# lixilinx/psgd_tf

Hardware: AMD Instinct MI355X
Metric: uvd_update_apply_params_per_sec (higher is better)
Workload: dtype f32

## Files before the change

### psgd_tf_amd/csrc/psgd_uvd.hip

```cpp
#include "uvd_kernels.h"
#include "psgd_hip.h"
#include <math.h>

namespace psgd {

const UvdOps* uvd_ops_group0(int r);
const UvdOps* uvd_ops_group1(int r);
const UvdOps* uvd_ops_group2(int r);
const UvdOps* uvd_ops_group3(int r);

const UvdWideOps* uvd_wide_group0(int r);
const UvdWideOps* uvd_wide_group1(int r);
const UvdWideOps* uvd_wide_group2(int r);
const UvdWideOps* uvd_wide_group3(int r);
const UvdWideOps* uvd_wide_ops_for_rank(int r) {
  if (r <= PSGD_UVD_MAX_RANK || r > 2 * PSGD_UVD_MAX_RANK) return nullptr;
  switch ((r - 33) / 8) {
    case 0: return uvd_wide_group0(r);
    case 1: return uvd_wide_group1(r);
    case 2: return uvd_wide_group2(r);
    default: return uvd_wide_group3(r);
  }
}

// ... 42 lines not shown
  double* sums; float* coef; float* maxbuf; void* part; float* pmax; float* nabla;
};

static int ws_open(void* ws, int64_t ws_bytes, int64_t N, int r, Ws* out) {
  if (N <= 0) return PSGD_ERR_BAD_ARG;
  if (r < 1 || r > PSGD_UVD_MAX_RANK) return PSGD_ERR_RANK;
  if (!ws || (reinterpret_cast<uintptr_t>(ws) & 255)) return PSGD_ERR_WORKSPACE;
  const WsLayout L = ws_layout(N, r);
  if (ws_bytes < L.total) return PSGD_ERR_WORKSPACE;
  char* b = static_cast<char*>(ws);
  out->sums = reinterpret_cast<double*>(b + L.sums_off);
  out->coef = reinterpret_cast<float*>(b + L.coef_off);
  out->maxbuf = reinterpret_cast<float*>(b + L.max_off);
  out->part = b + L.part_off;
  out->pmax = reinterpret_cast<float*>(b + L.pmax_off);
  out->nabla = reinterpret_cast<float*>(b + L.nabla_off);
  return PSGD_OK;
}

static inline bool misaligned16(const void* p) { return (reinterpret_cast<uintptr_t>(p) & 15) != 0; }

static int g_tune_staging = 0;
static int g_tune_blocks_per_cu = 0;
static int g_tune_tiles_per_wave = 8;

constexpr int kProfSlots = 8;
constexpr int kProfMaxPairs = 4096;
struct ProfPair { hipEvent_t e0, e1; };
static int g_prof_on = 0;
static ProfPair g_prof_pairs[kProfSlots][kProfMaxPairs];
static int g_prof_created[kProfSlots];
static int g_prof_used[kProfSlots];

struct ProfScope {
  hipEvent_t e1 = nullptr;
  hipStream_t st;
  ProfScope(int slot, hipStream_t s) : st(s) {
    if (!g_prof_on || slot < 0 || slot >= kProfSlots || g_prof_used[slot] >= kProfMaxPairs) return;
    const int i = g_prof_used[slot];
    if (i >= g_prof_created[slot]) {
      if (hipEventCreate(&g_prof_pairs[slot][i].e0) != hipSuccess) return;
      if (hipEventCreate(&g_prof_pairs[slot][i].e1) != hipSuccess) return;
      g_prof_created[slot] = i + 1;
    }
    g_prof_used[slot] = i + 1;
    (void)hipEventRecord(g_prof_pairs[slot][i].e0, st);
    e1 = g_prof_pairs[slot][i].e1;
  }
  ~ProfScope() {
    if (e1) (void)hipEventRecord(e1, st);
  }
};

static int num_cus() {
  static int n = 0;
  if (n == 0) {
    int dev = 0;
    (void)hipGetDevice(&dev);
    int v = 0;
    if (hipDeviceGetAttribute(&v, hipDeviceAttributeMultiprocessorCount, dev) != hipSuccess || v <= 0) v = 256;
    n = v;
  }
  return n;
}

static inline int use_nt(int64_t N, int r) {
  if (g_tune_staging == 1) return 0;
  if (g_tune_staging == 2) return 1;
  return (int64_t)N * r * 8 > (int64_t)192 * 1024 * 1024;
}

int policy_nt(int64_t stream_bytes) {
  if (g_tune_staging == 1) return 0;
  if (g_tune_staging == 2) return 1;
  return stream_bytes > (int64_t)192 * 1024 * 1024;
}
int policy_grid_blocks(int occ) {
  if (occ <= 0) occ = 1;
  if (g_tune_blocks_per_cu > 0 && g_tune_blocks_per_cu < occ) occ = g_tune_blocks_per_cu;
  if (g_tune_blocks_per_cu < 0) occ = -g_tune_blocks_per_cu;
  return occ;
}
int device_cus() { return num_cus(); }

static int g_tune_grid[16] = {0};

static int sweep_grid(const UvdOps* ops, int r, int which, int64_t N, int hard_cap) {
  static int occ_cache[PSGD_UVD_MAX_RANK + 1][16];
  if (which >= 0 && which < 16 && g_tune_grid[which] > 0) {
    const int64_t tiles = (N + ops->tile_rows - 1) / ops->tile_rows;
    int64_t grid = (tiles + kWavesPerBlock - 1) / kWavesPerBlock;
    if (grid > g_tune_grid[which]) grid = g_tune_grid[which];
    if (grid > hard_cap) grid = hard_cap;
    return (int)(grid < 1 ? 1 : grid);
  }
  int occ = occ_cache[r][which];
  if (occ == 0) {
    occ = ops->occupancy(which);
    if (occ <= 0) occ = 1;
    occ_cache[r][which] = occ;
  }
  if (which == kOccUpdS2U || which == kOccUpdS2V || which == kOccUpdS2F) {
    const int want = ((long)ops->tile_rows * r * 4 >= 4096) ? 1 : 2;
    if (want < occ) occ = want;
  } else if (which == kOccFinal) {
    occ = 1;
  }
  if (g_tune_blocks_per_cu > 0 && g_tune_blocks_per_cu < occ) occ = g_tune_blocks_per_cu;
  if (g_tune_blocks_per_cu < 0) occ = -g_tune_blocks_per_cu;
  const int64_t tiles = (N + ops->tile_rows - 1) / ops->tile_rows;
  int64_t grid = (tiles + kWavesPerBlock - 1) / kWavesPerBlock;
  int64_t cap = (int64_t)num_cus() * occ;
  if (g_tune_blocks_per_cu == 0) {
    int64_t want = tiles / (kWavesPerBlock * (g_tune_tiles_per_wave > 0 ? g_tune_tiles_per_wave : 1));
    if (want < num_cus()) want = num_cus();
    if (cap > want) cap = want;
  }
  if (grid > cap) grid = cap;
  if (grid > hard_cap) grid = hard_cap;
  if (grid < 1) grid = 1;
  return (int)grid;
}

template <class T>
__global__ __launch_bounds__(kThreads) void k_reduce_sum(const T* __restrict__ part, int G, int L,
                                                         double* __restrict__ sums, float* __restrict__ coef) {
  __shared__ double red[kWavesPerBlock][64];
  const int lane = threadIdx.x & 63, w = threadIdx.x >> 6;
  const int id = blockIdx.x * 64 + lane;
  double s = 0.0;
  if (id < L) {
    int b = w;
    for (; b + 7 * kWavesPerBlock < G; b += 8 * kWavesPerBlock) {
      T x[8];
#pragma unroll
      for (int u = 0; u < 8; ++u) x[u] = part[(long)(b + u * kWavesPerBlock) * L + id];
#pragma unroll
      for (int u = 0; u < 8; ++u) s += (double)x[u];
    }
    for (; b < G; b += kWavesPerBlock) s += (double)part[(long)b * L + id];
  }
  red[w][lane] = s;
  __syncthreads();
  if (w == 0 && id < L) {
    const double t = ((red[0][lane] + red[1][lane]) + red[2][lane]) + red[3][lane];
    sums[id] = t;
    if (coef) coef[id] = (float)t;
  }
}

__global__ __launch_bounds__(kThreads) void k_reduce_sum_t(const float* __restrict__ part, int G, int L,
                                                           double* __restrict__ sums, float* __restrict__ coef) {
  const int lane = threadIdx.x & 63;
  const int id = blockIdx.x * kWavesPerBlock + (threadIdx.x >> 6);
  if (id >= L) return;
  const float* p = part + (long)id * G;
  float x[kMaxGrid / 64];
#pragma unroll
  for (int u = 0; u < kMaxGrid / 64; ++u) x[u] = p[min(lane + 64 * u, G - 1)];
  double s = 0.0;
#pragma unroll
  for (int u = 0; u < kMaxGrid / 64; ++u) s += (lane + 64 * u < G) ? (double)x[u] : 0.0;
#pragma unroll
  for (int off = 32; off > 0; off >>= 1) s += __shfl_down(s, off, 64);
  if (lane == 0) {
    sums[id] = s;
// ... 655 lines not shown
      for (int off = 32; off > 0; off >>= 1) sum += __shfl_down(sum, off, 64);
      if (lane == 0) { pqs[e] = sum; pq[e] = sum; }
    }
  } else {
    for (int e = tid; e < 4 * r; e += blockDim.x) pqs[e] = pq[e];
    if (tid == 0) mx = maxbuf[0];
  }
  const int nb = (2 * r + 2 + 15) / 16;
  auto Gm = [&](int a, int b) -> double {
    if constexpr (DENSE) return gram[a * (2 * r + 2) + b];
    if (a > b) { const int t = a; a = b; b = t; }
    const int bi = a >> 4, bj = b >> 4, i = a & 15, j = b & 15;
    const int p = bi * nb - (bi * (bi - 1)) / 2 + (bj - bi);
    return gram[p * 256 + (i & 3) * 64 + (((i >> 2) << 4) | j)];
  };
  const bool act = tid < r;
  if (act) {
    for (int j0 = 0; j0 < r; j0 += 8) {
      double t[8];
#pragma unroll
      for (int u = 0; u < 8; ++u) t[u] = Gm(tid, (j0 + u < r) ? j0 + u : 0);
#pragma unroll
      for (int u = 0; u < 8; ++u)
        if (j0 + u < r) A[tid][j0 + u] = t[u];
    }
    if (update_U) {
      const double mu = c64[4 * r], aa = c64[4 * r + 1], ab = c64[4 * r + 2], bb = c64[4 * r + 3];
      const double Ua = c64[tid], Ub = c64[r + tid], c1 = c64[2 * r + tid], c2 = c64[3 * r + tid];
      for (int j = 0; j < r; ++j) {
        const double Uaj = c64[j], Ubj = c64[r + j], c1j = c64[2 * r + j], c2j = c64[3 * r + j];
        A[tid][j] += -mu * (Ua * c1j + c1 * Uaj - Ub * c2j - c2 * Ubj) +
                     mu * mu * (aa * c1 * c1j - ab * (c1 * c2j + c2 * c1j) + bb * c2 * c2j);
      }
    }
  }
  __syncthreads();
  const double mud = (double)(step / (mx + tiny));
  if (act) s1n[tid] = pqs[r + tid] - mud * pqs[3 * r + tid];
  __syncthreads();
  if (act) {
    double s2 = pqs[tid] - mud * pqs[2 * r + tid];
    for (int k = 0; k < r; ++k) s2 += A[tid][k] * s1n[k];
    coef[tid] = (float)s1n[tid];
    coef[r + tid] = (float)s2;
    s_out[tid] = s1n[tid];
    s_out[r + tid] = s2;
  }
}

}

using namespace psgd;

#define PSGD_CHECK_LAUNCH(expr)                 \
  do {                                          \
    const int _e = (expr);                      \
    if (_e != 0) return PSGD_ERR_LAUNCH;        \
  } while (0)

static inline int last_launch() { return (int)hipGetLastError(); }

extern "C" {

int psgd_abi_version(void) { return PSGD_ABI_VERSION; }

const char* psgd_error_string(int code) {
  switch (code) {
    case PSGD_OK: return "ok";
    case PSGD_ERR_BAD_ARG: return "bad argument (null pointer or non-positive size)";
    case PSGD_ERR_RANK: return "rank of modification outside [1, 32]";
    case PSGD_ERR_WORKSPACE: return "workspace missing, too small or not 256-byte aligned";
    case PSGD_ERR_ALIGN: return "matrix pointer not 16-byte aligned";
    case PSGD_ERR_LAUNCH: return "HIP kernel launch failed";
    case PSGD_ERR_SHAPE: return "inconsistent or unsupported matrix shapes";
    default: return "unknown error";
  }
}

int psgd_set_tuning(int key, int value) {
  if (key == 0) { g_tune_staging = value; return PSGD_OK; }
  if (key == 1) { g_tune_blocks_per_cu = value; return PSGD_OK; }
  if (key == 2) { g_tune_coef = value; return PSGD_OK; }
  if (key == 3) { g_tune_tiles_per_wave = value; return PSGD_OK; }
  if (key >= 10 && key < 26) { g_tune_grid[key - 10] = value; return PSGD_OK; }
  return PSGD_ERR_BAD_ARG;
}

int psgd_prof_enable(int on) {
  g_prof_on = on ? 1 : 0;
  for (int s = 0; s < kProfSlots; ++s) g_prof_used[s] = 0;
  return PSGD_OK;
}

int psgd_prof_collect(int slot, double* total_ms, int* count) {
  if (slot < 0 || slot >= kProfSlots || !total_ms || !count) return PSGD_ERR_BAD_ARG;
  double tot = 0.0;
  int n = 0;
  for (int i = 0; i < g_prof_used[slot]; ++i) {
    float ms = 0.0f;
    if (hipEventSynchronize(g_prof_pairs[slot][i].e1) != hipSuccess) continue;
    if (hipEventElapsedTime(&ms, g_prof_pairs[slot][i].e0, g_prof_pairs[slot][i].e1) != hipSuccess) continue;
    tot += ms;
    ++n;
  }
  g_prof_used[slot] = 0;
  *total_ms = tot;
  *count = n;
  return PSGD_OK;
}

int64_t psgd_uvd_workspace_bytes(int64_t N, int r) {
  if (N <= 0) return PSGD_ERR_BAD_ARG;
  if (r < 1 || r > PSGD_UVD_MAX_RANK) return PSGD_ERR_RANK;
  return ws_layout(N, r).total;
}

int psgd_uvd_ws_region(int which, int stage, int64_t N, int r, int64_t* offset_bytes, int64_t* count) {
  if (!offset_bytes || !count || N <= 0) return PSGD_ERR_BAD_ARG;
  if (r < 1 || r > PSGD_UVD_MAX_RANK) return PSGD_ERR_RANK;
  const WsLayout L = ws_layout(N, r);
  const int nc = 2 * r + 2, nb = (nc + 15) / 16, np = nb * (nb + 1) / 2;
  if (which == PSGD_WS_SUMS_F64) {
    if (stage == 1) { *offset_bytes = L.sums_off; *count = r; return PSGD_OK; }
    if (stage == 2) { *offset_bytes = L.sums_off + (int64_t)r * 8; *count = r; return PSGD_OK; }
    if (stage == 11) { *offset_bytes = L.sums_off; *count = (int64_t)np * 256; return PSGD_OK; }
    if (stage == 13) { *offset_bytes = L.sums_off + (int64_t)kPqSumsOff * 8; *count = 4 * r; return PSGD_OK; }
  } else if (which == PSGD_WS_MAX_F32) {
    if (stage == 10) { *offset_bytes = L.max_off; *count = 2; return PSGD_OK; }
    if (stage == 12) { *offset_bytes = L.max_off + 8; *count = 1; return PSGD_OK; }
  } else if (which == PSGD_WS_SEND_F64) {
    if (stage == 1 || stage == 2 || stage == 11) return psgd_uvd_ws_region(PSGD_WS_SUMS_F64, stage, N, r, offset_bytes, count);
    if (stage == 10) { *offset_bytes = L.sums_off + (int64_t)kBalD64Off * 8; *count = 2; return PSGD_OK; }
    if (stage == 12) { *offset_bytes = L.sums_off + (int64_t)(kPqSumsOff + 4 * r) * 8; *count = 1; return PSGD_OK; }
    if (stage == 13) { *offset_bytes = L.sums_off + (int64_t)kPqSumsOff * 8; *count = 4 * r + 1; return PSGD_OK; }
  }
  return PSGD_ERR_BAD_ARG;
}

int psgd_uvd_fold_gathered_f64(int stage, const double* gathered, int world, int64_t N, int r, void* ws,
                               int64_t ws_bytes, void* stream) {
  if (!gathered || world < 1) return PSGD_ERR_BAD_ARG;
  Ws w;
  const int rc = ws_open(ws, ws_bytes, N, r, &w);
  if (rc) return rc;
  int64_t off = 0, count = 0;
  const int rr = psgd_uvd_ws_region(PSGD_WS_SEND_F64, stage, N, r, &off, &count);
  if (rr) return rr;
  double* dst = reinterpret_cast<double*>(static_cast<char*>(ws) + off);
  int nsum = (int)count;
  float* maxdst = nullptr;
  if (stage == 10) { nsum = 0; maxdst = w.maxbuf; }
  else if (stage == 12) { nsum = 0; maxdst = w.maxbuf + 2; }
  else if (stage == 13) { nsum = 4 * r; maxdst = w.maxbuf + 2; }
  hipLaunchKernelGGL(k_fold_gathered, dim3(((int)count + 255) / 256), dim3(256), 0, static_cast<hipStream_t>(stream),
                     gathered, world, (int)count, nsum, dst, maxdst);
  PSGD_CHECK_LAUNCH(last_launch());
  return PSGD_OK;
}

int psgd_uvd_apply_sweep1_f32(const float* V, const float* d, const float* g, int64_t N, int r, void* ws,
                              int64_t ws_bytes, void* stream) {
  if (!V || !d || !g) return PSGD_ERR_BAD_ARG;
  Ws w;
  const int rc = ws_open(ws, ws_bytes, N, r, &w);
  if (rc) return rc;
  if (misaligned16(V)) return PSGD_ERR_ALIGN;
// ... 688 lines not shown
```

### psgd_tf_amd/csrc/uvd_kernels.h

```cpp
#pragma once
#include <hip/hip_runtime.h>
#include <stdint.h>
#include <type_traits>
#include "nanmax.h"

namespace psgd {

constexpr int kWave = 64;
constexpr int kWavesPerBlock = 4;
constexpr int kThreads = kWave * kWavesPerBlock;
constexpr int kMaxGrid = 2048;
constexpr int kGramMaxGrid = 1024;
#ifndef PSGD_TILE_CHUNK
#define PSGD_TILE_CHUNK 1
#endif
constexpr int kTileChunk = PSGD_TILE_CHUNK;

typedef float f32x4 __attribute__((ext_vector_type(4)));

#ifndef PSGD_WAVE_ID_VGPR
__device__ __forceinline__ int wave_in_block() { return __builtin_amdgcn_readfirstlane((int)(threadIdx.x >> 6)); }
#else
__device__ __forceinline__ int wave_in_block() { return (int)(threadIdx.x >> 6); }
#endif
// ... 862 lines not shown
    sweep_rows<R, 2, NV, (UPDATE_U ? 0 : 1), NT>(mats, vecs, UPDATE_U ? U : V, N, lds, body);
  }
  block_max_store(vmax, red, part_max + blockIdx.x);
}

template <int R, bool NT>
__global__ __launch_bounds__(kThreads) void k_uvd_final(const float* U, const float* V, float* d, const float* nabla,
                                                        const float* g, float* out, long N,
                                                        const float* __restrict__ coef, const float* __restrict__ maxbuf,
                                                        float step, float tiny) {
  __shared__ __attribute__((aligned(16))) float lds[kWavesPerBlock][sweep_lds_floats<R, 2, 3>()];
  const float mu = step / (maxbuf[0] + tiny);
  const float* const mats[2] = {U, V};
  const float* const vecs[3] = {d, nabla, g};
  sweep_rows<R, 2, 3, -1, NT>(mats, vecs, nullptr, N, lds[wave_in_block()],
                              [&](long row, bool valid, float (&x)[2][R], float (&s)[3]) {
                                const float dn = s[0] - (mu * s[0]) * s[1];
                                const float g1 = dn * s[2] + dot_row<R>(x[0], coef);
                                const float o = dn * (g1 + dot_row<R>(x[1], coef + R));
                                if (valid) {
                                  stream_store<NT>(d + row, dn);
                                  stream_store<NT>(out + row, o);
                                }
                              });
}

template <int R, bool NT, bool STR = false>
__global__ __launch_bounds__(kThreads) void k_rank2_update(float* M, const float* a, const float* b, long N,
                                                           const float* __restrict__ coef, long ld = R) {
  __shared__ __attribute__((aligned(16))) float lds[kWavesPerBlock][sweep_lds_floats<R, 1, 2>()];
  const float* const mats[1] = {M};
  const float* const vecs[2] = {a, b};
  sweep_rows<R, 1, 2, 0, NT, STR>(mats, vecs, M, N, lds[wave_in_block()],
                                  [&](long, bool, float (&x)[1][R], float (&s)[2]) {
#pragma unroll
                                    for (int c = 0; c < R; ++c) x[0][c] = x[0][c] - (s[0] * coef[c] - s[1] * coef[R + c]);
                                  }, NoTileHook(), RowStrides{{ld, ld}});
}

struct UvdOps {
  int tile_rows;
  int gram_len;
  int (*colreduce)(int nt, int nvec, const float* M, const float* a, const float* b, long N, float* part, int grid, hipStream_t st);
  int (*apply_s2)(int nt, const float* U, const float* d, const float* g, float* g1out, long N, const float* coef, float* part, int grid, hipStream_t st);
  int (*apply_s3)(int nt, const float* V, const float* d, float* out, long N, const float* coef, int grid, hipStream_t st);
  int (*rowdot_axpy)(int nt, const float* M, const float* x, float* out, long N, const float* coef, int grid, hipStream_t st);
  int (*update_gram)(int nt, const float* U, const float* V, const float* d, const float* v, const float* h, long N, double* part, int grid, hipStream_t st);
  int (*update_s2)(int nt, int update_U, float* U, float* V, const float* d, const float* v, const float* h, const float* g, long N, const float* coef, float* nabla, float* part_max, double* part_pq, int grid, hipStream_t st);
  int (*colreduce4)(int nt, const float* M, const float* const* x, long N, double* part, int grid, hipStream_t st);
  int (*rowdot_axpy4)(int nt, const float* M, const float* const* x, float* const* o, int ncols, long N, const float* coef, int grid, hipStream_t st);
  int (*rank2_update)(int nt, float* M, const float* a, const float* b, long N, const float* coef, int grid, hipStream_t st);
  int (*final_sweep)(int nt, const float* U, const float* V, float* d, const float* nabla, const float* g, float* out, long N, const float* coef, const float* maxbuf, float step, float tiny, int grid, hipStream_t st);
  int (*apply4_s1)(int nt, const float* V, const float* d, const float* const* x, long N, double* part, int grid, hipStream_t st);
  int (*apply4_s2)(int nt, const float* U, const float* d, const float* const* x, float* const* o, int ncols, long N, const float* coef, double* part, int grid, hipStream_t st);
  int (*apply4_s3)(int nt, const float* V, const float* d, float* const* o, int ncols, long N, const float* coef, int grid, hipStream_t st);
  int load_vec;
  int (*update_gram_ld)(const float* U, long ldU, const float* V, long ldV, const float* d, const float* v, const float* h, long N, double* part, int grid, hipStream_t st);
  int (*colreduce4_ld)(const float* M, long ld, const float* const* x, long N, double* part, int grid, hipStream_t st);
  int (*rowdot_axpy4_ld)(const float* M, long ld, const float* const* x, float* const* o, int ncols, long N, const float* coef, int grid, hipStream_t st);
  int (*rank2_update_ld)(float* M, long ld, const float* a, const float* b, long N, const float* coef, int grid, hipStream_t st);
  int (*occupancy)(int which);
};

struct UvdWideOps {
  int tile_rows;
  int (*colreduce4)(int nt, const float* M, const float* const* x, long N, double* part, int grid, hipStream_t st);
  int (*rowdot_axpy4)(int nt, const float* M, const float* const* x, float* const* o, int ncols, long N, const float* coef, int grid, hipStream_t st);
  int (*rank2_update)(int nt, float* M, const float* a, const float* b, long N, const float* coef, int grid, hipStream_t st);
  int (*apply4_s1)(int nt, const float* V, const float* d, const float* const* x, long N, double* part, int grid, hipStream_t st);
  int (*apply4_s2)(int nt, const float* U, const float* d, const float* const* x, float* const* o, int ncols, long N, const float* coef, double* part, int grid, hipStream_t st);
  int (*apply4_s3)(int nt, const float* V, const float* d, float* const* o, int ncols, long N, const float* coef, int grid, hipStream_t st);
  int (*update_s2)(int nt, int update_U, float* U, float* V, const float* d, const float* v, const float* h, const float* g, long N, const float* coef, float* nabla, float* part_max, double* part_pq, int grid, hipStream_t st);
  int (*final_sweep)(int nt, const float* U, const float* V, float* d, const float* nabla, const float* g, float* out, long N, const float* coef, const float* maxbuf, float step, float tiny, int grid, hipStream_t st);
};
const UvdWideOps* uvd_wide_ops_for_rank(int r);

enum { kOccColreduce = 0, kOccApplyS2, kOccApplyS3, kOccRowdot, kOccGram, kOccUpdS2U, kOccUpdS2V, kOccUpdS2F, kOccFinal };

const UvdOps* uvd_ops_for_rank(int r);

int policy_nt(int64_t stream_bytes);
int policy_grid_blocks(int occupancy);
int device_cus();

}
```

### psgd_tf_amd/csrc/uvd_wide_gram.hip

```cpp
#include "uvd_kernels.h"

#include "psgd_hip.h"

#include <cstdlib>

namespace psgd {

#ifndef GW_ACC64_LDS
#define GW_ACC64_LDS 0
#endif
#ifndef GW_DBG
#define GW_DBG 0
#endif
constexpr int kGwRows = 32;
constexpr int kGwThreads = 1024;
constexpr int kGwMulWaves = 11;
constexpr int kGwDepth = 4;

__host__ __device__ constexpr int gw_pair_index(int NB, int bi, int bj) { return bi * NB - (bi * (bi - 1)) / 2 + (bj - bi); }

struct GwPlan {
  int owner[15];
  int slot0[15];
  int max_load;
  int base[kGwMulWaves];
  int load[kGwMulWaves];
};
template <int NB>
constexpr GwPlan gw_make_plan() {
  constexpr int NS = (NB + 1) / 2, NSP = NS * (NS + 1) / 2;
  GwPlan p{};
  int load[kGwMulWaves] = {};
  int wt[15] = {};
  bool placed[15] = {};
  for (int si = 0; si < NS; ++si)
    for (int sj = si; sj < NS; ++sj) {
      const int na = (NB - 2 * si) < 2 ? (NB - 2 * si) : 2, nb = (NB - 2 * sj) < 2 ? (NB - 2 * sj) : 2;
      wt[gw_pair_index(NS, si, sj)] = si == sj ? na * (na + 1) / 2 : na * nb;
    }
  for (int round = 0; round < NSP; ++round) {
    int best = -1;
    for (int sp = 0; sp < NSP; ++sp)
      if (!placed[sp] && (best < 0 || wt[sp] > wt[best])) best = sp;
    int w = 0;
    for (int k = 1; k < kGwMulWaves; ++k)
      if (load[k] < load[w]) w = k;
    p.owner[best] = w;
    p.slot0[best] = load[w];
    load[w] += wt[best];
    placed[best] = true;
  }
  for (int k = 0; k < kGwMulWaves; ++k)
    if (load[k] > p.max_load) p.max_load = load[k];
  for (int k = 0, b = 0; k < kGwMulWaves; ++k) { p.base[k] = b; p.load[k] = load[k]; b += load[k]; }
  return p;
}
template <int NB> struct GwPlanOf { static constexpr GwPlan value = gw_make_plan<NB>(); };

template <int N> struct GwInt { static constexpr int value = N; };
template <int I, int N, class F>
__device__ __forceinline__ void gw_static_for(F&& f) {
  if constexpr (I < N) {
    f(GwInt<I>{});
    gw_static_for<I + 1, N>(f);
  }
}

#ifndef GW_UNIT_COLMAJOR
template <int NC> __device__ __forceinline__ int gw_unit(int col, int rg) { return rg * NC + col; }
#else
template <int NC> __device__ __forceinline__ int gw_unit(int col, int rg) { return col * 4 + (rg ^ ((col >> 2) & 2)); }
#endif

template <int NB, bool NT, bool TAIL>
__global__ __launch_bounds__(kGwThreads) void k_gram_wide(const float* __restrict__ U, const float* __restrict__ V,
                                                          const float* __restrict__ d, const float* __restrict__ v,
                                                          const float* __restrict__ h, long N, int r, long ntiles, long tile0,
                                                          double* __restrict__ part) {
  constexpr int NC = NB * 16;
  constexpr int NPW = GwPlanOf<NB>::value.max_load;
  constexpr int NP = NB * (NB + 1) / 2;
  typedef unsigned int u32x4g __attribute__((ext_vector_type(4)));
  __shared__ __attribute__((aligned(16))) u32x4g PL[2][3][NC * 4 + 16];
#if GW_ACC64_LDS
  __shared__ double A64[NP][4][64];
#endif
  const int tid = threadIdx.x, lane = tid & 63, wave = tid >> 6;
  const long G = gridDim.x;
  const long tfirst = TAIL ? tile0 : (long)blockIdx.x;
  if (TAIL) ntiles = tile0 + 1;

  const long nmine = (ntiles - tfirst + G - 1) / G;
  const long tlast = tfirst + (nmine - 1) * G;
  auto clampt = [&](long t) { return t < tlast ? t : tlast; };
  auto tile_loop = [&](auto&& prologue, auto&& step) {
    __syncthreads();
    prologue();
    __syncthreads();
    for (long i = 0; i < nmine; i += kGwDepth)
      gw_static_for<0, kGwDepth>([&](auto ic) {
        step(ic, tfirst + (i + decltype(ic)::value) * G);
        __syncthreads();
      });
  };
  if (wave < 4) {
    const int col = tid % r, g0 = tid / r;
    const bool on = g0 < 4;
    const unsigned e0 = on ? (unsigned)(g0 * 8 * r + col) : 0u;
    const unsigned eb0 = e0 * 4u;
    const int un0 = gw_unit<NC>(col, on ? g0 : 0), un1 = gw_unit<NC>(r + col, on ? g0 : 0);
    for (int i = tid; i < 2 * 3 * (NC * 4 + 16); i += 256) (&PL[0][0][0])[i] = u32x4g{0u, 0u, 0u, 0u};
    float px[kGwDepth][16];
    auto fetch = [&](long t, auto ic) {
      constexpr int ib = decltype(ic)::value;
      if constexpr (!TAIL) {
        const long toff0 = t * kGwRows * r;
        const long toff = ((long)__builtin_amdgcn_readfirstlane((int)(toff0 >> 32)) << 32) |
                          (unsigned)__builtin_amdgcn_readfirstlane((int)toff0);
        const unsigned tbytes = (unsigned)(kGwRows * r * 4);
        const auto ru = __builtin_amdgcn_make_buffer_rsrc(const_cast<float*>(U + toff), 0, tbytes, 0x00020000);
        const auto rv = __builtin_amdgcn_make_buffer_rsrc(const_cast<float*>(V + toff), 0, tbytes, 0x00020000);
        constexpr int aux = NT ? 2 : 0;
#pragma unroll
        for (int j = 0; j < 8; ++j) {
          px[ib][j] = __builtin_bit_cast(float, __builtin_amdgcn_raw_buffer_load_b32(ru, eb0, j * r * 4, aux));
          px[ib][8 + j] = __builtin_bit_cast(float, __builtin_amdgcn_raw_buffer_load_b32(rv, eb0, j * r * 4, aux));
        }
      } else {
        const long row0 = t * kGwRows + (on ? g0 : 0) * 8;
#pragma unroll
        for (int j = 0; j < 8; ++j) {
          const long row = row0 + j, rc = (row < N ? row : N - 1) * r + col;
          const float xu = stream_load<NT>(U + rc), xv = stream_load<NT>(V + rc);
          px[ib][j] = (on && row < N) ? xu : 0.0f;
          px[ib][8 + j] = (on && row < N) ? xv : 0.0f;
        }
      }
    };
    auto split_to = [&](int buf, auto ic) {
      constexpr int ib = decltype(ic)::value;
      if (GW_DBG & 4) {
#pragma unroll
        for (int j = 0; j < 16; ++j) asm volatile("" ::"v"(px[ib][j]));
        return;
      }
      if (!on) return;
      bf16x8 fh, fm, fl;
      float x[8];
#pragma unroll
      for (int hh = 0; hh < 2; ++hh) {
#pragma unroll
        for (int j = 0; j < 8; ++j) x[j] = px[ib][hh * 8 + j];
        split3_bf16(x, fh, fm, fl);
        const int un = hh ? un1 : un0;
        PL[buf][0][un] = __builtin_bit_cast(u32x4g, fh);
        PL[buf][1][un] = __builtin_bit_cast(u32x4g, fm);
        PL[buf][2][un] = __builtin_bit_cast(u32x4g, fl);
      }
    };
    const long t0 = tfirst;
    tile_loop(
        [&]() {
          gw_static_for<0, kGwDepth>([&](auto ic) { fetch(clampt(t0 + decltype(ic)::value * G), ic); });
          split_to(0, GwInt<0>{});
          fetch(clampt(t0 + kGwDepth * G), GwInt<0>{});
        },
        [&](auto ic, long t) {
          constexpr int q = decltype(ic)::value, slot = (q + 1) % kGwDepth;
          split_to((q + 1) & 1, GwInt<slot>{});
          fetch(clampt(t + (1 + kGwDepth) * G), GwInt<slot>{});
        });
    return;
  }
  if (wave == 4) {
    float* TW = reinterpret_cast<float*>(&PL[1][2][NC * 4]);
    const int tw_un = gw_unit<NC>(2 * r + (lane & 1), (lane >> 1) & 3);
    float pd[kGwDepth], ph[kGwDepth], pv[kGwDepth];
    bool pok[kGwDepth];
    const int it = lane >> 3;
    auto fetch = [&](long t, auto ic) {
      const long row = t * kGwRows + (it >> 1) * 8 + (lane & 7), rc = (!TAIL || row < N) ? row : N - 1;
      pd[decltype(ic)::value] = d[rc];
      ph[decltype(ic)::value] = h[rc];
      pv[decltype(ic)::value] = v[rc];
      pok[decltype(ic)::value] = !TAIL || row < N;
    };
    auto split_to = [&](int b, auto ic) {
      const float dd = pd[decltype(ic)::value], hh = ph[decltype(ic)::value], vv = pv[decltype(ic)::value];
      if (GW_DBG & 8) {
        asm volatile("" ::"v"(dd), "v"(hh), "v"(vv));
        return;
      }
      const float val = (it & 1) ? vv / dd : dd * hh;
      TW[lane] = pok[decltype(ic)::value] ? val : 0.0f;
      asm volatile("s_waitcnt lgkmcnt(0)" ::: "memory");
      __builtin_amdgcn_wave_barrier();
      if (lane < 8) {
        float x[8];
#pragma unroll
        for (int j = 0; j < 8; ++j) x[j] = TW[lane * 8 + j];
        bf16x8 fh, fm, fl;
        split3_bf16(x, fh, fm, fl);
        PL[b][0][tw_un] = __builtin_bit_cast(u32x4g, fh);
        PL[b][1][tw_un] = __builtin_bit_cast(u32x4g, fm);
        PL[b][2][tw_un] = __builtin_bit_cast(u32x4g, fl);
      }
      asm volatile("s_waitcnt lgkmcnt(0)" ::: "memory");
      __builtin_amdgcn_wave_barrier();
    };
    const long t0 = tfirst;
    tile_loop(
        [&]() {
          gw_static_for<0, kGwDepth>([&](auto ic) { fetch(clampt(t0 + decltype(ic)::value * G), ic); });
          split_to(0, GwInt<0>{});
          fetch(clampt(t0 + kGwDepth * G), GwInt<0>{});
        },
        [&](auto ic, long t) {
          constexpr int q = decltype(ic)::value, slot = (q + 1) % kGwDepth;
          split_to((q + 1) & 1, GwInt<slot>{});
          fetch(clampt(t + (1 + kGwDepth) * G), GwInt<slot>{});
        });
    return;
  }
  const int mw = wave - 5;
  f32x4 acc[NPW];
#if GW_ACC64_LDS
  int my_base = 0, my_load = 0;
  gw_static_for<0, kGwMulWaves>([&](auto kc) {
    if (mw == decltype(kc)::value) { my_base = GwPlanOf<NB>::value.base[decltype(kc)::value]; my_load = GwPlanOf<NB>::value.load[decltype(kc)::value]; }
  });
  double (*my64)[4][64] = A64 + my_base;
#pragma unroll
  for (int p = 0; p < NPW; ++p) {
    acc[p] = f32x4{0.f, 0.f, 0.f, 0.f};
    if (p < my_load)
#pragma unroll
      for (int e = 0; e < 4; ++e) my64[p][e][lane] = 0.0;
  }
  auto fold = [&]() {
#pragma unroll
    for (int p = 0; p < NPW; ++p) {
      if (p < my_load)
#pragma unroll
        for (int e = 0; e < 4; ++e) my64[p][e][lane] += (double)acc[p][e];
      acc[p] = f32x4{0.f, 0.f, 0.f, 0.f};
    }
  };
#else
  double acc64[NPW][4];
#pragma unroll
  for (int p = 0; p < NPW; ++p) {
    acc[p] = f32x4{0.f, 0.f, 0.f, 0.f};
#pragma unroll
    for (int e = 0; e < 4; ++e) acc64[p][e] = 0.0;
  }
  auto fold = [&]() {
#pragma unroll
    for (int p = 0; p < NPW; ++p) {
#pragma unroll
      for (int e = 0; e < 4; ++e) acc64[p][e] += (double)acc[p][e];
      acc[p] = f32x4{0.f, 0.f, 0.f, 0.f};
    }
  };
#endif
  int since = 0;
  tile_loop([]() {}, [&](auto ic, long t) {
    if (t >= ntiles) return;
    const int buf = decltype(ic)::value & 1;
    auto frag = [&](int b, bf16x8 (&f)[3]) {
      const int un = gw_unit<NC>(b * 16 + (lane & 15), lane >> 4);
#pragma unroll
      for (int pl = 0; pl < 3; ++pl) f[pl] = __builtin_bit_cast(bf16x8, PL[buf][pl][un]);
    };
    constexpr int NS = (NB + 1) / 2;
    gw_static_for<0, NS>([&](auto sic) {
      constexpr int si = decltype(sic)::value;
      gw_static_for<si, NS>([&](auto sjc) {
        constexpr int sj = decltype(sjc)::value;
        constexpr int sp = gw_pair_index(NS, si, sj);
        constexpr int own = GwPlanOf<NB>::value.owner[sp], s0 = GwPlanOf<NB>::value.slot0[sp];
        constexpr int na = (NB - 2 * si) < 2 ? (NB - 2 * si) : 2, nb = (NB - 2 * sj) < 2 ? (NB - 2 * sj) : 2;
        if (mw == own && !(GW_DBG & 2)) {
          bf16x8 fa[2][3], fb[2][3];
          gw_static_for<0, nb>([&](auto c) { frag(2 * sj + decltype(c)::value, fb[decltype(c)::value]); });
          if constexpr (si != sj) gw_static_for<0, na>([&](auto c) { frag(2 * si + decltype(c)::value, fa[decltype(c)::value]); });
          gw_static_for<0, 6>([&](auto tc) {
            constexpr int term = decltype(tc)::value;
            constexpr int pa = term == 0 ? 1 : term == 1 ? 0 : term == 2 ? 2 : term == 3 ? 0 : term == 4 ? 1 : 0;
            constexpr int pb = term == 0 ? 1 : term == 1 ? 2 : term == 2 ? 0 : term == 3 ? 1 : term == 4 ? 0 : 0;
            gw_static_for<0, na>([&](auto ac) {
              constexpr int a = decltype(ac)::value;
              gw_static_for<(si == sj ? a : 0), nb>([&](auto bc) {
                constexpr int b = decltype(bc)::value;
                constexpr int slot = s0 + (si == sj ? (a == 0 ? b : nb + (b - 1)) : a * nb + b);
                if constexpr (si == sj) acc[slot] = __builtin_amdgcn_mfma_f32_16x16x32_bf16(fb[a][pa], fb[b][pb], acc[slot], 0, 0, 0);
                else acc[slot] = __builtin_amdgcn_mfma_f32_16x16x32_bf16(fa[a][pa], fb[b][pb], acc[slot], 0, 0, 0);
              });
            });
          });
        }
      });
    });
    if (++since == 256 / kGwRows) {
      fold();
      since = 0;
    }
  });
  fold();
  double* dst = part + (long)blockIdx.x * NP * 256;
  {
    constexpr int NS = (NB + 1) / 2;
    gw_static_for<0, NS>([&](auto sic) {
      constexpr int si = decltype(sic)::value;
      gw_static_for<si, NS>([&](auto sjc) {
        constexpr int sj = decltype(sjc)::value;
        constexpr int sp = gw_pair_index(NS, si, sj);
        constexpr int own = GwPlanOf<NB>::value.owner[sp], s0 = GwPlanOf<NB>::value.slot0[sp];
        constexpr int na = (NB - 2 * si) < 2 ? (NB - 2 * si) : 2, nb = (NB - 2 * sj) < 2 ? (NB - 2 * sj) : 2;
        if (mw == own) {
          gw_static_for<0, na>([&](auto ac) {
            constexpr int a = decltype(ac)::value;
            gw_static_for<(si == sj ? a : 0), nb>([&](auto bc) {
              constexpr int b = decltype(bc)::value;
              constexpr int slot = s0 + (si == sj ? (a == 0 ? b : nb + (b - 1)) : a * nb + b);
              constexpr int pi = gw_pair_index(NB, 2 * si + a, 2 * sj + b);
#pragma unroll
#if GW_ACC64_LDS
              for (int e = 0; e < 4; ++e) dst[pi * 256 + e * 64 + lane] = my64[slot][e][lane];
#else
              for (int e = 0; e < 4; ++e) dst[pi * 256 + e * 64 + lane] = acc64[slot][e];
#endif
            });
          });
        }
      });
    });
  }
}

__global__ __launch_bounds__(kThreads) void k_gram_wide_finish(const double* __restrict__ part, int nblocks, int NB, int ncol,
                                                               double* __restrict__ G) {
  const int NP = NB * (NB + 1) / 2;
  const int idx = blockIdx.x * kThreads + threadIdx.x;
  if (idx >= NP * 256) return;
  const int p = idx >> 8, q = idx & 255, e = q >> 6, l = q & 63;
  int bi = 0, rem = p;
  while (rem >= NB - bi) { rem -= NB - bi; ++bi; }
  const int bj = bi + rem;
  double s = 0.0;
  const double* src = part + (long)p * 256 + q;
  const long st = (long)NP * 256;
  int b = 0;
  for (; b + 8 <= nblocks; b += 8) {
    double x[8];
#pragma unroll
    for (int u = 0; u < 8; ++u) x[u] = src[(b + u) * st];
#pragma unroll
    for (int u = 0; u < 8; ++u) s += x[u];
  }
  for (; b < nblocks; ++b) s += src[b * st];
  const int i = 16 * bi + 4 * (l >> 4) + e, j = 16 * bj + (l & 15);
  if (i < ncol && j < ncol && (bi != bj || i <= j)) {
    G[(long)i * ncol + j] = s;
    G[(long)j * ncol + i] = s;
  }
}

template <int NB>
static int launch_gram_wide(int nt, const float* U, const float* V, const float* d, const float* v, const float* h, long N, int r,
                            double* part, int grid, hipStream_t st) {
  const long nfull = N / kGwRows;
  if (nfull > 0) {
    if (nt) hipLaunchKernelGGL((k_gram_wide<NB, true, false>), dim3(grid), dim3(kGwThreads), 0, st, U, V, d, v, h, N, r, nfull, 0L, part);
    else hipLaunchKernelGGL((k_gram_wide<NB, false, false>), dim3(grid), dim3(kGwThreads), 0, st, U, V, d, v, h, N, r, nfull, 0L, part);
    if (hipGetLastError() != hipSuccess) return 1;
  }
  if (N % kGwRows) {
    double* tail = part + (long)(nfull > 0 ? grid : 0) * (NB * (NB + 1) / 2) * 256;
    hipLaunchKernelGGL((k_gram_wide<NB, false, true>), dim3(1), dim3(kGwThreads), 0, st, U, V, d, v, h, N, r, nfull + 1, nfull, tail);
  }
  return (int)hipGetLastError();
}

}

using namespace psgd;

static int gram_wide_grid(int64_t N) {
  const int64_t tiles = N / kGwRows;
  int64_t g = (int64_t)device_cus();
  if (g > tiles) g = tiles;
  if (g < 1) g = 1;
  return (int)g;
}

extern "C" {

int64_t psgd_uvd_gram_wide_scratch_bytes(int64_t N, int r) {
  if (N <= 0 || r <= PSGD_UVD_MAX_RANK || r > 2 * PSGD_UVD_MAX_RANK) return PSGD_ERR_RANK;
  const int NB = (2 * r + 2 + 15) / 16;
  return (int64_t)(gram_wide_grid(N) + 1) * (NB * (NB + 1) / 2) * 256 * 8;
}

int psgd_uvd_gram_wide_f32(const float* U, const float* V, const float* d, const float* v, const float* h, int64_t N, int r,
                           double* G, void* scratch, int64_t scratch_bytes, void* stream) {
  if (!U || !V || !d || !v || !h || !G || N <= 0) return PSGD_ERR_BAD_ARG;
  if (r <= PSGD_UVD_MAX_RANK || r > 2 * PSGD_UVD_MAX_RANK) return PSGD_ERR_RANK;
  const int64_t need = psgd_uvd_gram_wide_scratch_bytes(N, r);
  if (!scratch || (reinterpret_cast<uintptr_t>(scratch) & 255) || scratch_bytes < need) return PSGD_ERR_WORKSPACE;
  hipStream_t st = static_cast<hipStream_t>(stream);
  const int NB = (2 * r + 2 + 15) / 16, grid = gram_wide_grid(N);
  static const int env_nt = getenv("PSGD_GW_NT") ? atoi(getenv("PSGD_GW_NT")) : -1;
  const int nt = env_nt >= 0 ? env_nt : policy_nt(2 * N * r * 4);
  double* part = static_cast<double*>(scratch);
  int e = 1;
  switch (NB) {
    case 5: e = launch_gram_wide<5>(nt, U, V, d, v, h, N, r, part, grid, st); break;
    case 6: e = launch_gram_wide<6>(nt, U, V, d, v, h, N, r, part, grid, st); break;
    case 7: e = launch_gram_wide<7>(nt, U, V, d, v, h, N, r, part, grid, st); break;
    case 8: e = launch_gram_wide<8>(nt, U, V, d, v, h, N, r, part, grid, st); break;
    case 9: e = launch_gram_wide<9>(nt, U, V, d, v, h, N, r, part, grid, st); break;
    default: return PSGD_ERR_RANK;
  }
  if (e) return PSGD_ERR_LAUNCH;
  const int NP = NB * (NB + 1) / 2, ncol = 2 * r + 2;
  const int nsets = (N / kGwRows > 0 ? grid : 0) + (N % kGwRows ? 1 : 0);
  hipLaunchKernelGGL(k_gram_wide_finish, dim3((NP * 256 + kThreads - 1) / kThreads), dim3(kThreads), 0, st, part, nsets, NB, ncol, G);
  return hipGetLastError() == hipSuccess ? PSGD_OK : PSGD_ERR_LAUNCH;
}

}
```

Measured before the change: 9.725 billion.

## Use scaled two-term fp16 split for wide Gram MFMA instead of bf16x3

Adds a new default path for the wide-rank Gram kernel. Each column is scaled by a power of two taken from a per-column max over the tile, then split into fp16 hi and lo parts, and the Gram is built with three fp16 MFMA products per block pair instead of the bf16 three-way split. This cuts LDS planes from three to two and reduces the MFMA work. In exchange it adds max reductions, exponent bookkeeping in LDS, and per-element ldexp rescaling, with some risk to accuracy for columns with a wide dynamic range. The old bf16x3 path stays available through a tuning key.

```diff
diff --git a/psgd_tf_amd/csrc/psgd_uvd.hip b/psgd_tf_amd/csrc/psgd_uvd.hip
--- a/psgd_tf_amd/csrc/psgd_uvd.hip
+++ b/psgd_tf_amd/csrc/psgd_uvd.hip
@@ -148,6 +148,9 @@
   return occ;
 }
 int device_cus() { return num_cus(); }
+
+static int g_tune_gram_wide = 0;
+int policy_gram_wide_bf16x3() { return g_tune_gram_wide == 1; }
 
 static int g_tune_grid[16] = {0};
 
@@ -969,6 +972,7 @@
   if (key == 1) { g_tune_blocks_per_cu = value; return PSGD_OK; }
   if (key == 2) { g_tune_coef = value; return PSGD_OK; }
   if (key == 3) { g_tune_tiles_per_wave = value; return PSGD_OK; }
+  if (key == 4) { g_tune_gram_wide = value; return PSGD_OK; }
   if (key >= 10 && key < 26) { g_tune_grid[key - 10] = value; return PSGD_OK; }
   return PSGD_ERR_BAD_ARG;
 }
diff --git a/psgd_tf_amd/csrc/uvd_kernels.h b/psgd_tf_amd/csrc/uvd_kernels.h
--- a/psgd_tf_amd/csrc/uvd_kernels.h
+++ b/psgd_tf_amd/csrc/uvd_kernels.h
@@ -968,5 +968,6 @@
 int policy_nt(int64_t stream_bytes);
 int policy_grid_blocks(int occupancy);
 int device_cus();
-
-}
+int policy_gram_wide_bf16x3();
+
+}
diff --git a/psgd_tf_amd/csrc/uvd_wide_gram.hip b/psgd_tf_amd/csrc/uvd_wide_gram.hip
--- a/psgd_tf_amd/csrc/uvd_wide_gram.hip
+++ b/psgd_tf_amd/csrc/uvd_wide_gram.hip
@@ -72,7 +72,25 @@
 template <int NC> __device__ __forceinline__ int gw_unit(int col, int rg) { return col * 4 + (rg ^ ((col >> 2) & 2)); }
 #endif
 
-template <int NB, bool NT, bool TAIL>
+typedef _Float16 f16x8g __attribute__((ext_vector_type(8)));
+__device__ __forceinline__ int gw_scale_exp(unsigned maxbits) {
+  const int ef = (int)(maxbits >> 23);
+  if (maxbits == 0u || ef == 255) return 0;
+  const int e = 140 - ef;
+  return e < 126 ? e : 126;
+}
+__device__ __forceinline__ float gw_pow2(int e) { return __uint_as_float((unsigned)(e + 127) << 23); }
+__device__ __forceinline__ void split2_f16(const float (&x)[8], float s, f16x8g& h, f16x8g& M) {
+#pragma unroll
+  for (int j = 0; j < 8; ++j) {
+    const float xs = x[j] * s;
+    const _Float16 hj = (_Float16)xs;
+    h[j] = hj;
+    M[j] = (_Float16)((xs - (float)hj) * 2048.0f);
+  }
+}
+
+template <int NB, bool NT, bool TAIL, int FMT>
 __global__ __launch_bounds__(kGwThreads) void k_gram_wide(const float* __restrict__ U, const float* __restrict__ V,
                                                           const float* __restrict__ d, const float* __restrict__ v,
                                                           const float* __restrict__ h, long N, int r, long ntiles, long tile0,
@@ -81,7 +99,10 @@
   constexpr int NPW = GwPlanOf<NB>::value.max_load;
   constexpr int NP = NB * (NB + 1) / 2;
   typedef unsigned int u32x4g __attribute__((ext_vector_type(4)));
-  __shared__ __attribute__((aligned(16))) u32x4g PL[2][3][NC * 4 + 16];
+  constexpr int NPL = FMT ? 2 : 3;
+  __shared__ __attribute__((aligned(16))) u32x4g PL[2][NPL][NC * 4 + 16];
+  __shared__ __attribute__((aligned(16))) int EX[FMT ? 2 : 1][FMT ? NC : 4];
+  __shared__ unsigned MX[FMT ? 2 : 1][FMT ? 4 : 1][FMT ? NC : 1];
 #if GW_ACC64_LDS
   __shared__ double A64[NP][4][64];
 #endif
@@ -109,7 +130,9 @@
     const unsigned e0 = on ? (unsigned)(g0 * 8 * r + col) : 0u;
     const unsigned eb0 = e0 * 4u;
     const int un0 = gw_unit<NC>(col, on ? g0 : 0), un1 = gw_unit<NC>(r + col, on ? g0 : 0);
-    for (int i = tid; i < 2 * 3 * (NC * 4 + 16); i += 256) (&PL[0][0][0])[i] = u32x4g{0u, 0u, 0u, 0u};
+    for (int i = tid; i < 2 * NPL * (NC * 4 + 16); i += 256) (&PL[0][0][0])[i] = u32x4g{0u, 0u, 0u, 0u};
+    if constexpr (FMT == 1)
+      for (int i = tid; i < 2 * NC; i += 256) (&EX[0][0])[i] = 0;
     float px[kGwDepth][16];
     auto fetch = [&](long t, auto ic) {
       constexpr int ib = decltype(ic)::value;
@@ -145,20 +168,60 @@
         return;
       }
       if (!on) return;
-      bf16x8 fh, fm, fl;
       float x[8];
 #pragma unroll
       for (int hh = 0; hh < 2; ++hh) {
 #pragma unroll
         for (int j = 0; j < 8; ++j) x[j] = px[ib][hh * 8 + j];
-        split3_bf16(x, fh, fm, fl);
         const int un = hh ? un1 : un0;
-        PL[buf][0][un] = __builtin_bit_cast(u32x4g, fh);
-        PL[buf][1][un] = __builtin_bit_cast(u32x4g, fm);
-        PL[buf][2][un] = __builtin_bit_cast(u32x4g, fl);
+        if constexpr (FMT == 1) {
+          const int c = hh ? r + col : col;
+          const unsigned m01 = max(MX[buf][0][c], MX[buf][1][c]), m23 = max(MX[buf][2][c], MX[buf][3][c]);
+          const int e = gw_scale_exp(max(m01, m23));
+          f16x8g fh, fM;
+          split2_f16(x, gw_pow2(e), fh, fM);
+          PL[buf][0][un] = __builtin_bit_cast(u32x4g, fh);
+          PL[buf][1][un] = __builtin_bit_cast(u32x4g, fM);
+          if (g0 == 0) EX[buf][c] = -e;
+        } else {
+          bf16x8 fh, fm, fl;
+          split3_bf16(x, fh, fm, fl);
+          PL[buf][0][un] = __builtin_bit_cast(u32x4g, fh);
+          PL[buf][1][un] = __builtin_bit_cast(u32x4g, fm);
+          PL[buf][NPL - 1][un] = __builtin_bit_cast(u32x4g, fl);
+        }
       }
     };
     const long t0 = tfirst;
+    if constexpr (FMT == 1) {
+      auto pmax = [&](int par, auto ic) {
+        constexpr int ib = decltype(ic)::value;
+        if (!on) return;
+        unsigned mu = 0u, mv = 0u;
+#pragma unroll
+        for (int j = 0; j < 8; ++j) {
+          mu = max(mu, __float_as_uint(px[ib][j]) & 0x7FFFFFFFu);
+          mv = max(mv, __float_as_uint(px[ib][8 + j]) & 0x7FFFFFFFu);
+        }
+        MX[par][g0][col] = mu;
+        MX[par][g0][r + col] = mv;
+      };
+      gw_static_for<0, kGwDepth>([&](auto ic) { fetch(clampt(t0 + decltype(ic)::value * G), ic); });
+      pmax(0, GwInt<0>{});
+      tile_loop(
+          [&]() {
+            split_to(0, GwInt<0>{});
+            fetch(clampt(t0 + kGwDepth * G), GwInt<0>{});
+            pmax(1, GwInt<1 % kGwDepth>{});
+          },
+          [&](auto ic, long t) {
+            constexpr int q = decltype(ic)::value, slot = (q + 1) % kGwDepth;
+            split_to((q + 1) & 1, GwInt<slot>{});
+            fetch(clampt(t + (1 + kGwDepth) * G), GwInt<slot>{});
+            pmax(q & 1, GwInt<(q + 2) % kGwDepth>{});
+          });
+      return;
+    }
     tile_loop(
         [&]() {
           gw_static_for<0, kGwDepth>([&](auto ic) { fetch(clampt(t0 + decltype(ic)::value * G), ic); });
@@ -173,7 +236,7 @@
     return;
   }
   if (wave == 4) {
-    float* TW = reinterpret_cast<float*>(&PL[1][2][NC * 4]);
+    float* TW = reinterpret_cast<float*>(&PL[1][NPL - 1][NC * 4]);
     const int tw_un = gw_unit<NC>(2 * r + (lane & 1), (lane >> 1) & 3);
     float pd[kGwDepth], ph[kGwDepth], pv[kGwDepth];
     bool pok[kGwDepth];
@@ -191,19 +254,36 @@
         asm volatile("" ::"v"(dd), "v"(hh), "v"(vv));
         return;
       }
-      const float val = (it & 1) ? vv / dd : dd * hh;
-      TW[lane] = pok[decltype(ic)::value] ? val : 0.0f;
+      float val = (it & 1) ? vv / dd : dd * hh;
+      val = pok[decltype(ic)::value] ? val : 0.0f;
+      if constexpr (FMT == 1) {
+        unsigned mb = __float_as_uint(val) & 0x7FFFFFFFu;
+#pragma unroll
+        for (int o = 1; o < 64; o <<= 1)
+          if (o != 8) mb = max(mb, (unsigned)__shfl_xor((int)mb, o));
+        const int e = gw_scale_exp(mb);
+        val *= gw_pow2(e);
+        if ((lane & ~8) == 0) EX[b][2 * r + (lane >> 3)] = -e;
+      }
+      TW[lane] = val;
       asm volatile("s_waitcnt lgkmcnt(0)" ::: "memory");
       __builtin_amdgcn_wave_barrier();
       if (lane < 8) {
         float x[8];
 #pragma unroll
         for (int j = 0; j < 8; ++j) x[j] = TW[lane * 8 + j];
-        bf16x8 fh, fm, fl;
-        split3_bf16(x, fh, fm, fl);
-        PL[b][0][tw_un] = __builtin_bit_cast(u32x4g, fh);
-        PL[b][1][tw_un] = __builtin_bit_cast(u32x4g, fm);
-        PL[b][2][tw_un] = __builtin_bit_cast(u32x4g, fl);
+        if constexpr (FMT == 1) {
+          f16x8g fh, fM;
+          split2_f16(x, 1.0f, fh, fM);
+          PL[b][0][tw_un] = __builtin_bit_cast(u32x4g, fh);
+          PL[b][1][tw_un] = __builtin_bit_cast(u32x4g, fM);
+        } else {
+          bf16x8 fh, fm, fl;
+          split3_bf16(x, fh, fm, fl);
+          PL[b][0][tw_un] = __builtin_bit_cast(u32x4g, fh);
+          PL[b][1][tw_un] = __builtin_bit_cast(u32x4g, fm);
+          PL[b][NPL - 1][tw_un] = __builtin_bit_cast(u32x4g, fl);
+        }
       }
       asm volatile("s_waitcnt lgkmcnt(0)" ::: "memory");
       __builtin_amdgcn_wave_barrier();
@@ -264,6 +344,64 @@
   };
 #endif
   int since = 0;
+  if constexpr (FMT == 1) {
+    tile_loop([]() {}, [&](auto ic, long t) {
+      if (t >= ntiles) return;
+      const int buf = decltype(ic)::value & 1;
+      auto frag = [&](int b, f16x8g (&f)[2]) {
+        const int un = gw_unit<NC>(b * 16 + (lane & 15), lane >> 4);
+#pragma unroll
+        for (int pl = 0; pl < 2; ++pl) f[pl] = __builtin_bit_cast(f16x8g, PL[buf][pl][un]);
+      };
+      typedef int i32x4g __attribute__((ext_vector_type(4)));
+      constexpr int NS = (NB + 1) / 2;
+      gw_static_for<0, NS>([&](auto sic) {
+        constexpr int si = decltype(sic)::value;
+        gw_static_for<si, NS>([&](auto sjc) {
+          constexpr int sj = decltype(sjc)::value;
+          constexpr int sp = gw_pair_index(NS, si, sj);
+          constexpr int own = GwPlanOf<NB>::value.owner[sp], s0 = GwPlanOf<NB>::value.slot0[sp];
+          constexpr int na = (NB - 2 * si) < 2 ? (NB - 2 * si) : 2, nb = (NB - 2 * sj) < 2 ? (NB - 2 * sj) : 2;
+          if (mw == own && !(GW_DBG & 2)) {
+            f16x8g fa[2][2], fb[2][2];
+            int ej[2];
+            gw_static_for<0, nb>([&](auto c) {
+              frag(2 * sj + decltype(c)::value, fb[decltype(c)::value]);
+              ej[decltype(c)::value] = EX[buf][(2 * sj + decltype(c)::value) * 16 + (lane & 15)];
+            });
+            if constexpr (si != sj) gw_static_for<0, na>([&](auto c) { frag(2 * si + decltype(c)::value, fa[decltype(c)::value]); });
+            gw_static_for<0, na>([&](auto ac) {
+              constexpr int a = decltype(ac)::value;
+              constexpr int b0 = si == sj ? a : 0;
+              const i32x4g ei = *reinterpret_cast<const i32x4g*>(&EX[buf][(2 * si + a) * 16 + 4 * (lane >> 4)]);
+              f32x4 H[2], X[2];
+              gw_static_for<b0, nb>([&](auto bc) { H[decltype(bc)::value] = X[decltype(bc)::value] = f32x4{0.f, 0.f, 0.f, 0.f}; });
+              gw_static_for<0, 3>([&](auto tc) {
+                constexpr int term = decltype(tc)::value;
+                gw_static_for<b0, nb>([&](auto bc) {
+                  constexpr int b = decltype(bc)::value;
+                  const f16x8g ah = si == sj ? fb[a][0] : fa[a][0], aM = si == sj ? fb[a][1] : fa[a][1];
+                  if constexpr (term == 0) X[b] = __builtin_amdgcn_mfma_f32_16x16x32_f16(aM, fb[b][0], X[b], 0, 0, 0);
+                  if constexpr (term == 1) H[b] = __builtin_amdgcn_mfma_f32_16x16x32_f16(ah, fb[b][0], H[b], 0, 0, 0);
+                  if constexpr (term == 2) X[b] = __builtin_amdgcn_mfma_f32_16x16x32_f16(ah, fb[b][1], X[b], 0, 0, 0);
+                });
+              });
+              gw_static_for<b0, nb>([&](auto bc) {
+                constexpr int b = decltype(bc)::value;
+                constexpr int slot = s0 + (si == sj ? (a == 0 ? b : nb + (b - 1)) : a * nb + b);
+#pragma unroll
+                for (int e = 0; e < 4; ++e) acc[slot][e] += ldexpf(fmaf(X[b][e], 0x1p-11f, H[b][e]), ei[e] + ej[b]);
+              });
+            });
+          }
+        });
+      });
+      if (++since == 256 / kGwRows) {
+        fold();
+        since = 0;
+      }
+    });
+  } else
   tile_loop([]() {}, [&](auto ic, long t) {
     if (t >= ntiles) return;
     const int buf = decltype(ic)::value & 1;
@@ -366,18 +504,18 @@
   }
 }
 
-template <int NB>
+template <int NB, int FMT>
 static int launch_gram_wide(int nt, const float* U, const float* V, const float* d, const float* v, const float* h, long N, int r,
                             double* part, int grid, hipStream_t st) {
   const long nfull = N / kGwRows;
   if (nfull > 0) {
-    if (nt) hipLaunchKernelGGL((k_gram_wide<NB, true, false>), dim3(grid), dim3(kGwThreads), 0, st, U, V, d, v, h, N, r, nfull, 0L, part);
-    else hipLaunchKernelGGL((k_gram_wide<NB, false, false>), dim3(grid), dim3(kGwThreads), 0, st, U, V, d, v, h, N, r, nfull, 0L, part);
+    if (nt) hipLaunchKernelGGL((k_gram_wide<NB, true, false, FMT>), dim3(grid), dim3(kGwThreads), 0, st, U, V, d, v, h, N, r, nfull, 0L, part);
+    else hipLaunchKernelGGL((k_gram_wide<NB, false, false, FMT>), dim3(grid), dim3(kGwThreads), 0, st, U, V, d, v, h, N, r, nfull, 0L, part);
     if (hipGetLastError() != hipSuccess) return 1;
   }
   if (N % kGwRows) {
     double* tail = part + (long)(nfull > 0 ? grid : 0) * (NB * (NB + 1) / 2) * 256;
-    hipLaunchKernelGGL((k_gram_wide<NB, false, true>), dim3(1), dim3(kGwThreads), 0, st, U, V, d, v, h, N, r, nfull + 1, nfull, tail);
+    hipLaunchKernelGGL((k_gram_wide<NB, false, true, FMT>), dim3(1), dim3(kGwThreads), 0, st, U, V, d, v, h, N, r, nfull + 1, nfull, tail);
   }
   return (int)hipGetLastError();
 }
@@ -413,13 +551,14 @@
   static const int env_nt = getenv("PSGD_GW_NT") ? atoi(getenv("PSGD_GW_NT")) : -1;
   const int nt = env_nt >= 0 ? env_nt : policy_nt(2 * N * r * 4);
   double* part = static_cast<double*>(scratch);
+  const bool bf16x3 = policy_gram_wide_bf16x3() != 0;
   int e = 1;
   switch (NB) {
-    case 5: e = launch_gram_wide<5>(nt, U, V, d, v, h, N, r, part, grid, st); break;
-    case 6: e = launch_gram_wide<6>(nt, U, V, d, v, h, N, r, part, grid, st); break;
-    case 7: e = launch_gram_wide<7>(nt, U, V, d, v, h, N, r, part, grid, st); break;
-    case 8: e = launch_gram_wide<8>(nt, U, V, d, v, h, N, r, part, grid, st); break;
-    case 9: e = launch_gram_wide<9>(nt, U, V, d, v, h, N, r, part, grid, st); break;
+    case 5: e = bf16x3 ? launch_gram_wide<5, 0>(nt, U, V, d, v, h, N, r, part, grid, st) : launch_gram_wide<5, 1>(nt, U, V, d, v, h, N, r, part, grid, st); break;
+    case 6: e = bf16x3 ? launch_gram_wide<6, 0>(nt, U, V, d, v, h, N, r, part, grid, st) : launch_gram_wide<6, 1>(nt, U, V, d, v, h, N, r, part, grid, st); break;
+    case 7: e = bf16x3 ? launch_gram_wide<7, 0>(nt, U, V, d, v, h, N, r, part, grid, st) : launch_gram_wide<7, 1>(nt, U, V, d, v, h, N, r, part, grid, st); break;
+    case 8: e = bf16x3 ? launch_gram_wide<8, 0>(nt, U, V, d, v, h, N, r, part, grid, st) : launch_gram_wide<8, 1>(nt, U, V, d, v, h, N, r, part, grid, st); break;
+    case 9: e = bf16x3 ? launch_gram_wide<9, 0>(nt, U, V, d, v, h, N, r, part, grid, st) : launch_gram_wide<9, 1>(nt, U, V, d, v, h, N, r, part, grid, st); break;
     default: return PSGD_ERR_RANK;
   }
   if (e) return PSGD_ERR_LAUNCH;
```

Result: no change. 9.739 billion, median of 6 (+0.1%).
